# henriChevreux/distillation_trajectories

Hardware: AMD Instinct MI355X
Metric: trajectory-timesteps/sec (B×T U-Net fwd) at 16×16 T=50 (higher is better)
Workload: dtype f32 (fp32-accurate; convolutions: exact 3-plane bf16 operand split on bf16 MFMA with fp32 accumulate, or native fp32 MFMA, chosen per layer)

## Files before the change

### distillation_trajectories_amd/csrc/dt_conv_strip.hip

```cpp
#include <mutex>
#include <type_traits>

#include "dt_conv_epilogue.h"

namespace dt {

extern __shared__ __attribute__((aligned(16))) __bf16 strip_lds[];

template <int BM, int BN, int ABL = 0, int KC = 1, int WK = 1>
__global__ __launch_bounds__(256, KC == 1 ? 3 : 2) void conv_strip_bf16x6_kernel(const ConvParams p) {
  constexpr int WN = WK > 1 ? BN / 64 : (BM == 256 ? 1 : 2), WM = 4 / (WN * WK), NT = 256;
  constexpr int MI = BM / (32 * WM), NI = BN / (32 * WN);
  constexpr int KW = KC / WK;
  static_assert(KC % WK == 0 && MI * 32 * WM == BM && NI * 32 * WN == BN && (WK == 1 || (MI == 2 && NI == 2)), "wave layout");
  constexpr int PLANE_B = BN * 16, STAGE_B = 3 * PLANE_B;
  constexpr int AP = BM == 256 ? 3 : (KC == 4 ? 1 : 2);
  const int halo = strip_halo(p.W, BM);
  const int R = BM + 2 * halo;
  const int RZ = (R + 7) & ~7;
  const int PLANE_A = (RZ + 8) * 16;
  __bf16 *As = strip_lds;
  __bf16 *Bs = strip_lds + KC * 3 * PLANE_A;

  const int tid = threadIdx.x, lane = tid & 63;
  const int wave = __builtin_amdgcn_readfirstlane(tid >> 6);
  const int wk = wave % WK, wm = (wave / WK) / WN, wn = (wave / WK) % WN;
  const int half = lane >> 5, l31 = lane & 31;
  const int m0 = blockIdx.x * BM, n0 = blockIdx.y * BN;
  const int HW = p.H * p.W;
  const int CC = p.cin_p >> 4;

  bool s_in[AP], s_ok[AP], s_core[AP];
  int s_off[AP], s_off2[AP], s_offb[AP], s_lds[AP];
#pragma unroll
  for (int i = 0; i < AP; ++i) {
    const int item = tid + i * NT;
    const int srow = item >> 1, hh = item & 1;
    const int m = m0 - halo + srow;
    s_in[i] = item < 2 * R;
    s_ok[i] = s_in[i] && m >= 0 && m < p.M;
    s_core[i] = s_ok[i] && srow >= halo && srow < halo + BM;
    const int mm = s_ok[i] ? m : 0;
    s_off[i] = mm * p.cin_p + hh * 8;
    s_off2[i] = mm * p.cin2_p + hh * 8;
    s_offb[i] = mm * p.b_stride + hh * 8;
    s_lds[i] = srow * 16 + ((hh ^ ((srow >> 3) & 1)) << 3);
  }
  constexpr bool B_ALL = WK > 1 && BN * 4 == NT;
  constexpr int NB = B_ALL ? KC * 3 / 2 : KC * 3, SB = B_ALL ? 2 : 1;
  static_assert(!B_ALL || (KC * 3) % 2 == 0, "weight staging");
  const bool b_thread = B_ALL || tid < BN * 2;
  const int bt = B_ALL ? (tid & (BN * 2 - 1)) : tid, bsub = B_ALL ? tid / (BN * 2) : 0;
  const size_t w_plane = (size_t)p.n_p * 16;
  const __bf16 *wbase = reinterpret_cast<const __bf16 *>(p.w) + (size_t)n0 * 16 + bt * 8 + bsub * w_plane;
  const __bf16 *wbase2 = reinterpret_cast<const __bf16 *>(p.w2) + (size_t)n0 * 16 + bt * 8 + bsub * w_plane;
  const int b_lds = bsub * PLANE_B + bt * 8;

  int a_row[MI];
  unsigned a_mask[MI];
#pragma unroll
  for (int mi = 0; mi < MI; ++mi) {
    const int row_i = wm * (MI * 32) + mi * 32 + l31;
    const int m = m0 + row_i;
    a_row[mi] = row_i + halo;
    unsigned mask = 0;
    if (m < p.M) {
      const int rem = m % HW;
      const int y = rem / p.W, x = rem - y * p.W;
#pragma unroll
      for (int t = 0; t < 9; ++t) {
        const int yy = y + t / 3 - 1, xx = x + t % 3 - 1;
        if (yy >= 0 && yy < p.H && xx >= 0 && xx < p.W) mask |= 1u << t;
      }
    }
    a_mask[mi] = mask;
  }
  int b_frag[NI];
#pragma unroll
  for (int ni = 0; ni < NI; ++ni) {
    const int row = wn * (NI * 32) + ni * 32 + l31;
    b_frag[ni] = row * 16 + ((half ^ ((row >> 3) & 1)) << 3);
  }

  f32x16 acc[MI][NI];
#pragma unroll
  for (int mi = 0; mi < MI; ++mi)
#pragma unroll
    for (int ni = 0; ni < NI; ++ni)
#pragma unroll
      for (int r = 0; r < 16; ++r) acc[mi][ni][r] = 0.f;

  const int n_main = (CC + p.splits * KC - 1) / (p.splits * KC);
  const int cc0 = blockIdx.z * n_main * KC;
  const int CC2 = p.cin2_p >> 4;
  const int n_chunks = n_main + (p.in2 ? (CC2 + KC - 1) / KC : 0);

  f32x4 sa0[KC][AP], sa1[KC][AP];
  u32x4 rb[NB];
  auto load_strip = [&](int ch) __attribute__((always_inline)) {
#pragma unroll
    for (int kk = 0; kk < KC; ++kk)
#pragma unroll
    for (int i = 0; i < AP; ++i) {
      sa0[kk][i] = f32x4{0.f, 0.f, 0.f, 0.f}; sa1[kk][i] = sa0[kk][i];
      if (ch < n_main) {
        const int cc = cc0 + ch * KC + kk;
        if (s_ok[i] && cc < CC) {
          const float *src = (p.in_b && cc >= p.cc_a) ? p.in_b + s_offb[i] + (cc - p.cc_a) * 16 : p.in + s_off[i] + cc * 16;
          sa0[kk][i] = *reinterpret_cast<const f32x4 *>(src);
          sa1[kk][i] = *reinterpret_cast<const f32x4 *>(src + 4);
        }
      } else if (s_core[i] && (ch - n_main) * KC + kk < CC2) {
        const int c2 = (ch - n_main) * KC + kk;
        const float *src = (p.in2_b && c2 >= p.cc_a) ? p.in2_b + s_offb[i] + (c2 - p.cc_a) * 16 : p.in2 + s_off2[i] + c2 * 16;
        sa0[kk][i] = *reinterpret_cast<const f32x4 *>(src);
        sa1[kk][i] = *reinterpret_cast<const f32x4 *>(src + 4);
      }
    }
  };
  auto write_strip = [&]() __attribute__((always_inline)) {
#pragma unroll
    for (int kk = 0; kk < KC; ++kk)
#pragma unroll
    for (int i = 0; i < AP; ++i)
      if (s_in[i]) {
        bf16x8 p1, p2, p3;
        split8(sa0[kk][i], sa1[kk][i], p1, p2, p3);
        __bf16 *A = As + kk * 3 * PLANE_A;
        *reinterpret_cast<bf16x8 *>(A + s_lds[i]) = p1;
        *reinterpret_cast<bf16x8 *>(A + PLANE_A + s_lds[i]) = p2;
        *reinterpret_cast<bf16x8 *>(A + 2 * PLANE_A + s_lds[i]) = p3;
      }
  };
  const size_t tap_stride = (size_t)p.ccw * 3 * w_plane, group_stride = (size_t)KC * 3 * w_plane;
  const __bf16 *wrun = wbase + (size_t)cc0 * 3 * w_plane;
  enum { ADV_NONE = 0, ADV_TAP, ADV_GROUP, ADV_SKIP0, ADV_SKIP };
  auto load_b = [&](int adv) __attribute__((always_inline)) {
    if (adv == ADV_TAP) wrun += tap_stride;
    else if (adv == ADV_GROUP) wrun = wrun - 8 * tap_stride + group_stride;
    else if (adv == ADV_SKIP0) wrun = wbase2;
    else if (adv == ADV_SKIP) wrun += group_stride;
    if (b_thread) {
      const __bf16 *wt = ABL == 6 ? wbase : wrun;
#pragma unroll
      for (int i = 0; i < NB; ++i)
        rb[i] = *reinterpret_cast<const u32x4 *>(wt + (SB * i) * w_plane);
    }
  };
  auto write_b = [&](int stage) __attribute__((always_inline)) {
    if (b_thread) {
      __bf16 *B = Bs + stage * KC * STAGE_B;
#pragma unroll
      for (int i = 0; i < NB; ++i) *reinterpret_cast<u32x4 *>(B + (SB * i) * PLANE_B + b_lds) = rb[i];
    }
  };

  constexpr bool DB = WK > 1 && ABL == 0;
  bf16x8 fbn[KW][NI][3];
  auto load_bd = [&](int adv) __attribute__((always_inline)) {
    if (adv == ADV_TAP) wrun += tap_stride;
    else if (adv == ADV_GROUP) wrun = wrun - 8 * tap_stride + group_stride;
    else if (adv == ADV_SKIP0) wrun = wbase2;
    else if (adv == ADV_SKIP) wrun += group_stride;
    const __bf16 *wt = wrun - (bt * 8 + bsub * w_plane);
#pragma unroll
    for (int kw = 0; kw < KW; ++kw)
#pragma unroll
      for (int ni = 0; ni < NI; ++ni)
#pragma unroll
        for (int pl = 0; pl < 3; ++pl)
          fbn[kw][ni][pl] = *reinterpret_cast<const bf16x8 *>(wt + ((wk * KW + kw) * 3 + pl) * w_plane + b_frag[ni]);
  };

  const long long tl0 = p.ablate == 8 ? wall_clock64() : 0;
  load_strip(0);
  if (DB) load_bd(ADV_NONE); else load_b(ADV_NONE);
  if (tid < 48 * KC) *reinterpret_cast<u32x4 *>(As + (tid >> 4) * PLANE_A + RZ * 16 + (tid & 15) * 8) = u32x4{0u, 0u, 0u, 0u};
  write_strip();
  if (!DB) write_b(0);
  __syncthreads();

  unsigned long long ph[4] = {0, 0, 0, 0}, ts = 0;
  auto stamp = [&](int seg) __attribute__((always_inline)) {
    if (ABL != 9) return;
    unsigned long long t;
    __builtin_amdgcn_sched_barrier(0);
    asm volatile("s_memtime %0\n\ts_waitcnt lgkmcnt(0)" : "=s"(t) :: "memory");
    __builtin_amdgcn_sched_barrier(0);
    if (seg >= 0) ph[seg] += t - ts;
    ts = t;
  };
  stamp(-1);
  const long long tl_pro = p.ablate == 8 ? wall_clock64() : 0;
  int step = 0;
  bool stage_next_strip = true;
  auto do_step = [&](auto TT, int ch, bool first_tap, bool last_tap, bool next_chunk, int adv) __attribute__((always_inline)) {
    constexpr int tt = decltype(TT)::value;
    const bool more = !last_tap || next_chunk;
    if (first_tap && next_chunk && stage_next_strip && ABL != 5) load_strip(ch + 1);
    bf16x8 fbc[KW][NI][3];
    if (DB) {
#pragma unroll
      for (int kw = 0; kw < KW; ++kw)
#pragma unroll
        for (int ni = 0; ni < NI; ++ni)
#pragma unroll
          for (int pl = 0; pl < 3; ++pl) fbc[kw][ni][pl] = fbn[kw][ni][pl];
      if (more) load_bd(adv);
    } else if (more && ABL != 2) load_b(adv);
    {
      int wv = p.W;
      asm volatile("" : "+s"(wv));
      const int shift = (tt / 3 - 1) * wv + (tt % 3 - 1);
      int a_e[MI];
#pragma unroll
      for (int mi = 0; mi < MI; ++mi) {
        int row0 = a_row[mi];
        asm volatile("" : "+v"(row0));
        const int srow = row0 + shift;
        const int lrow = ((a_mask[mi] >> tt) & 1u) ? srow : RZ + (srow & 7);
        a_e[mi] = lrow * 16 + ((half ^ ((srow >> 3) & 1)) << 3);
      }
#pragma unroll
      for (int kw = 0; kw < KW; ++kw) {
        const int kk = wk * KW + kw;
        const __bf16 *A = As + kk * 3 * PLANE_A;
        const __bf16 *B = Bs + ((step & 1) * KC + kk) * STAGE_B;
        bf16x8 fb[NI][3];
        const u32x4 fake = {(unsigned)lane * 0x01010101u + (unsigned)a_e[0], 0x3f803f80u, (unsigned)step, 0x3c003c00u};
#pragma unroll
        for (int ni = 0; ni < NI; ++ni)
#pragma unroll
          for (int pl = 0; pl < 3; ++pl)
            fb[ni][pl] = DB ? fbc[kw][ni][pl]
                            : ((ABL == 4) ? __builtin_bit_cast(bf16x8, fake) : *reinterpret_cast<const bf16x8 *>(B + pl * PLANE_B + b_frag[ni]));
#pragma unroll
        for (int mi = 0; mi < MI; ++mi) {
          bf16x8 fa[3];
#pragma unroll
          for (int pl = 0; pl < 3; ++pl)
            fa[pl] = (ABL == 4) ? __builtin_bit_cast(bf16x8, fake) : *reinterpret_cast<const bf16x8 *>(A + pl * PLANE_A + a_e[mi]);
#pragma unroll
          for (int ni = 0; ni < NI; ++ni) {
            f32x16 c = acc[mi][ni];
            if (ABL == 3) {
              asm volatile("" :: "v"(fa[0]), "v"(fa[1]), "v"(fa[2]), "v"(fb[ni][0]), "v"(fb[ni][1]), "v"(fb[ni][2]));
              continue;
            }
            c = __builtin_amdgcn_mfma_f32_32x32x16_bf16(fa[2], fb[ni][0], c, 0, 0, 0);
            c = __builtin_amdgcn_mfma_f32_32x32x16_bf16(fa[1], fb[ni][1], c, 0, 0, 0);
            c = __builtin_amdgcn_mfma_f32_32x32x16_bf16(fa[0], fb[ni][2], c, 0, 0, 0);
            c = __builtin_amdgcn_mfma_f32_32x32x16_bf16(fa[1], fb[ni][0], c, 0, 0, 0);
            c = __builtin_amdgcn_mfma_f32_32x32x16_bf16(fa[0], fb[ni][1], c, 0, 0, 0);
            c = __builtin_amdgcn_mfma_f32_32x32x16_bf16(fa[0], fb[ni][0], c, 0, 0, 0);
            acc[mi][ni] = c;
          }
        }
      }
    }
    stamp(0);
    if (ABL == 9) { asm volatile("s_waitcnt vmcnt(0)" ::: "memory"); stamp(1); }
    if (!DB && more && ABL != 2) write_b((step + 1) & 1);
    stamp(2);
    const bool restage = last_tap && next_chunk && stage_next_strip && ABL != 5;
    if (restage) {
      __syncthreads();
      write_strip();
    }
    if (DB ? restage : (ABL != 1 || last_tap)) __syncthreads();
    stamp(3);
    ++step;
  };

  constexpr bool DIRECT = MI * KW <= 2 && KC >= 2 && ABL == 0;
  f32x4 ga0[KW][MI][2], ga1[KW][MI][2];
  const int n_skip = p.in2 ? (CC2 + KC - 1) / KC : 0;
  auto load_a = [&](f32x4 (&g)[KW][MI][2], int s2) __attribute__((always_inline)) {
#pragma unroll
    for (int kw = 0; kw < KW; ++kw)
#pragma unroll
      for (int mi = 0; mi < MI; ++mi) {
        const int c2 = s2 * KC + wk * KW + kw;
        const int m = m0 + wm * (MI * 32) + mi * 32 + l31;
        g[kw][mi][0] = f32x4{0.f, 0.f, 0.f, 0.f}; g[kw][mi][1] = g[kw][mi][0];
        if (m < p.M && c2 < CC2) {
          const float *src = (p.in2_b && c2 >= p.cc_a) ? p.in2_b + (size_t)m * p.b_stride + (c2 - p.cc_a) * 16 + half * 8
                                                       : p.in2 + (size_t)m * p.cin2_p + c2 * 16 + half * 8;
          g[kw][mi][0] = *reinterpret_cast<const f32x4 *>(src);
          g[kw][mi][1] = *reinterpret_cast<const f32x4 *>(src + 4);
        }
      }
  };
  auto skip_step = [&](f32x4 (&g)[KW][MI][2], int s2) __attribute__((always_inline)) {
    const bool more = s2 + 1 < n_skip;
    bf16x8 fbc[KW][NI][3];
    if (DB) {
#pragma unroll
      for (int kw = 0; kw < KW; ++kw)
#pragma unroll
        for (int ni = 0; ni < NI; ++ni)
#pragma unroll
          for (int pl = 0; pl < 3; ++pl) fbc[kw][ni][pl] = fbn[kw][ni][pl];
      if (more) load_bd(ADV_SKIP);
    } else if (more) load_b(ADV_SKIP);
#pragma unroll
    for (int kw = 0; kw < KW; ++kw) {
      const int kk = wk * KW + kw;
      const __bf16 *B = Bs + ((step & 1) * KC + kk) * STAGE_B;
      bf16x8 fb[NI][3];
#pragma unroll
      for (int ni = 0; ni < NI; ++ni)
#pragma unroll
        for (int pl = 0; pl < 3; ++pl) fb[ni][pl] = DB ? fbc[kw][ni][pl] : *reinterpret_cast<const bf16x8 *>(B + pl * PLANE_B + b_frag[ni]);
#pragma unroll
      for (int mi = 0; mi < MI; ++mi) {
        bf16x8 fa[3];
        split8(g[kw][mi][0], g[kw][mi][1], fa[0], fa[1], fa[2]);
#pragma unroll
        for (int ni = 0; ni < NI; ++ni) {
          f32x16 c = acc[mi][ni];
          c = __builtin_amdgcn_mfma_f32_32x32x16_bf16(fa[2], fb[ni][0], c, 0, 0, 0);
          c = __builtin_amdgcn_mfma_f32_32x32x16_bf16(fa[1], fb[ni][1], c, 0, 0, 0);
          c = __builtin_amdgcn_mfma_f32_32x32x16_bf16(fa[0], fb[ni][2], c, 0, 0, 0);
          c = __builtin_amdgcn_mfma_f32_32x32x16_bf16(fa[1], fb[ni][0], c, 0, 0, 0);
          c = __builtin_amdgcn_mfma_f32_32x32x16_bf16(fa[0], fb[ni][1], c, 0, 0, 0);
          c = __builtin_amdgcn_mfma_f32_32x32x16_bf16(fa[0], fb[ni][0], c, 0, 0, 0);
          acc[mi][ni] = c;
        }
      }
    }
    if (s2 + 2 < n_skip) load_a(g, s2 + 2);
    if (!DB) {
      if (more) write_b((step + 1) & 1);
      __syncthreads();
    }
    ++step;
  };

  const int prio_grp = ((blockIdx.x + gridDim.x * (blockIdx.y + gridDim.y * blockIdx.z)) >> 8) & 1;
  const bool use_prio = p.ablate != 7 && gridDim.x * gridDim.y * gridDim.z <= 512;
  for (int ch = 0; ch < n_main; ++ch) {
    if (use_prio) {
      if ((ch ^ prio_grp) & 1) __builtin_amdgcn_s_setprio(1);
      else __builtin_amdgcn_s_setprio(0);
    }
    const bool next_chunk = ch + 1 < ((WK > 1 && p.in2) ? n_main : n_chunks);
    if (DIRECT && WK == 1 && p.in2 && ch + 1 == n_main) {
      stage_next_strip = false;
      load_a(ga0, 0);
      if (n_skip > 1) load_a(ga1, 1);
    }
    do_step(std::integral_constant<int, 0>{}, ch, true, false, next_chunk, ADV_TAP);
    do_step(std::integral_constant<int, 1>{}, ch, false, false, next_chunk, ADV_TAP);
    do_step(std::integral_constant<int, 2>{}, ch, false, false, next_chunk, ADV_TAP);
    do_step(std::integral_constant<int, 3>{}, ch, false, false, next_chunk, ADV_TAP);
    do_step(std::integral_constant<int, 4>{}, ch, false, false, next_chunk, ADV_TAP);
    do_step(std::integral_constant<int, 5>{}, ch, false, false, next_chunk, ADV_TAP);
    do_step(std::integral_constant<int, 6>{}, ch, false, false, next_chunk, ADV_TAP);
    do_step(std::integral_constant<int, 7>{}, ch, false, false, next_chunk, ADV_TAP);
    do_step(std::integral_constant<int, 8>{}, ch, false, true, next_chunk, ch + 1 < n_main ? ADV_GROUP : ADV_SKIP0);
    if (ch + 1 == n_main && p.in2) {
      if constexpr (WK == 1) {
        conv_midpoint<MI, NI>(p, acc, n0, wn, l31);
      } else {
        constexpr int P = BN + 4, COPY = WM * 32 * P;
        float *red = reinterpret_cast<float *>(strip_lds);
#pragma unroll
        for (int mi = 0; mi < MI; ++mi) {
          if (mi || DB) __syncthreads();
#pragma unroll
          for (int ni = 0; ni < NI; ++ni)
#pragma unroll
            for (int r = 0; r < 16; ++r)
              red[wk * COPY + (wm * 32 + 4 * half + (r & 3) + 8 * (r >> 2)) * P + wn * (NI * 32) + ni * 32 + l31] = acc[mi][ni][r];
          __syncthreads();
#pragma unroll
          for (int ni = 0; ni < NI; ++ni)
#pragma unroll
            for (int r = 0; r < 16; ++r) {
              const float *src = red + (wm * 32 + 4 * half + (r & 3) + 8 * (r >> 2)) * P + wn * (NI * 32) + ni * 32 + l31;
              float v = src[0];
#pragma unroll
              for (int c = 1; c < WK; ++c) v += src[c * COPY];
              acc[mi][ni][r] = wk == 0 ? v : 0.f;
            }
        }
        if (wk == 0) conv_midpoint<MI, NI>(p, acc, n0, wn, l31);
        __syncthreads();
        if (DB) load_bd(ADV_SKIP0); else load_b(ADV_SKIP0);
        if (DIRECT) {
          load_a(ga0, 0);
          if (n_skip > 1) load_a(ga1, 1);
        } else {
          load_strip(n_main);
          if (tid < 48 * KC) *reinterpret_cast<u32x4 *>(As + (tid >> 4) * PLANE_A + RZ * 16 + (tid & 15) * 8) = u32x4{0u, 0u, 0u, 0u};
          write_strip();
        }
        if (!DB) write_b(step & 1);
        __syncthreads();
      }
    }
  }
  __builtin_amdgcn_s_setprio(0);
  if (DIRECT) {
    for (int s2 = 0; s2 < n_skip; s2 += 2) {
      skip_step(ga0, s2);
      if (s2 + 1 < n_skip) skip_step(ga1, s2 + 1);
    }
  } else {
    for (int ch = n_main; ch < n_chunks; ++ch)
      do_step(std::integral_constant<int, 4>{}, ch, true, true, ch + 1 < n_chunks, ADV_SKIP);
  }
  const long long tl1 = p.ablate == 8 ? wall_clock64() : 0;
  conv_epilogue<MI, NI, WM, WK>(p, acc, reinterpret_cast<float *>(strip_lds), m0, n0, wm, wn, half, l31, wk);
  if (ABL == 9) {
    if (lane == 0) {
      unsigned long long *rec = reinterpret_cast<unsigned long long *>(p.slab) + 8 * (4 * (blockIdx.x + gridDim.x * (blockIdx.y + gridDim.y * blockIdx.z)) + wave);
      rec[0] = ph[0]; rec[1] = ph[1]; rec[2] = ph[2]; rec[3] = ph[3]; rec[4] = (unsigned long long)step;
    }
  }
  if (p.ablate == 8 && p.splits == 1) {
    __syncthreads();
    if (tid == 0) {
      long long *rec = reinterpret_cast<long long *>(p.slab) + 4 * (blockIdx.x + gridDim.x * blockIdx.y);
      rec[0] = tl0; rec[1] = tl_pro; rec[2] = tl1; rec[3] = wall_clock64();
    }
  }
}

int launch_conv_strip(const ConvParams &p_in, hipStream_t s) {
  ConvParams p = p_in;
  const int bm = p.bm, bn = p.bn, kind = p.kind;
  const int kc = strip_kc(kind, bm, bn);
  dim3 grid((p.M + bm - 1) / bm, p.n_p / bn, p.splits);
  size_t lds = strip_lds_bytes(p.W, bm, bn, kind);
  p.dup_stage2 = 0;
  if (p.n_dup == 2 && p.pool_out) {
    const size_t rows1 = bm == 256 || kc == 4 || (kind == KIND_STRIPK && bm == 128) ? 128 : 64;
    const size_t rows2 = bm == 256 ? 128 : (bm == 128 ? 64 : 32);
    const size_t need = (rows1 + (kind == KIND_STRIPK ? rows2 : rows1)) * (bn + 4) * sizeof(float);
    if (need <= strip_lds_limit(kind)) {
      p.dup_stage2 = 1;
      if (need > lds) lds = need;
    }
  }
#ifdef DT_TOOLS
  if (p.ablate && p.ablate != 7 && p.ablate != 8 && bm == 128 && bn == 128) {
    switch (p.ablate) {
      case 1: conv_strip_bf16x6_kernel<128, 128, 1><<<grid, 256, lds, s>>>(p); break;
      case 2: conv_strip_bf16x6_kernel<128, 128, 2><<<grid, 256, lds, s>>>(p); break;
      case 3: conv_strip_bf16x6_kernel<128, 128, 3><<<grid, 256, lds, s>>>(p); break;
      case 4: conv_strip_bf16x6_kernel<128, 128, 4><<<grid, 256, lds, s>>>(p); break;
      case 5: conv_strip_bf16x6_kernel<128, 128, 5><<<grid, 256, lds, s>>>(p); break;
      case 6: conv_strip_bf16x6_kernel<128, 128, 6><<<grid, 256, lds, s>>>(p); break;
      case 9: conv_strip_bf16x6_kernel<128, 128, 9><<<grid, 256, lds, s>>>(p); break;
      default: return DT_E_ARG;
    }
    DT_LAUNCH_CHECK();
    return DT_OK;
  }
#endif
  if (kind != KIND_STRIP) {
    static std::once_flag attr_once;
    static int attr_status = DT_OK;
    std::call_once(attr_once, [] {
      const void *fns[8] = {reinterpret_cast<const void *>(&conv_strip_bf16x6_kernel<64, 128, 0, 2, 2>),
                            reinterpret_cast<const void *>(&conv_strip_bf16x6_kernel<64, 64, 0, 4, 4>),
                            reinterpret_cast<const void *>(&conv_strip_bf16x6_kernel<128, 64, 0, 2, 2>),
                            reinterpret_cast<const void *>(&conv_strip_bf16x6_kernel<256, 64, 0, 2>),
                            reinterpret_cast<const void *>(&conv_strip_bf16x6_kernel<128, 128, 0, 2>),
                            reinterpret_cast<const void *>(&conv_strip_bf16x6_kernel<128, 64, 0, 2>),
                            reinterpret_cast<const void *>(&conv_strip_bf16x6_kernel<64, 128, 0, 2>),
                            reinterpret_cast<const void *>(&conv_strip_bf16x6_kernel<64, 64, 0, 2>)};
      for (const void *f : fns) {
        const hipError_t e = hipFuncSetAttribute(f, hipFuncAttributeMaxDynamicSharedMemorySize, 98304);
        if (e != hipSuccess) attr_status = (int)e;
      }
    });
    if (attr_status != DT_OK) return attr_status;
    if (kind == KIND_STRIPK && bn == 128) conv_strip_bf16x6_kernel<64, 128, 0, 2, 2><<<grid, 256, lds, s>>>(p);
    else if (kind == KIND_STRIPK && bm == 64) conv_strip_bf16x6_kernel<64, 64, 0, 4, 4><<<grid, 256, lds, s>>>(p);
    else if (kind == KIND_STRIPK) conv_strip_bf16x6_kernel<128, 64, 0, 2, 2><<<grid, 256, lds, s>>>(p);
    else if (bm == 256) conv_strip_bf16x6_kernel<256, 64, 0, 2><<<grid, 256, lds, s>>>(p);
    else if (bm == 128 && bn == 128) conv_strip_bf16x6_kernel<128, 128, 0, 2><<<grid, 256, lds, s>>>(p);
    else if (bm == 128) conv_strip_bf16x6_kernel<128, 64, 0, 2><<<grid, 256, lds, s>>>(p);
    else if (bn == 128) conv_strip_bf16x6_kernel<64, 128, 0, 2><<<grid, 256, lds, s>>>(p);
    else conv_strip_bf16x6_kernel<64, 64, 0, 2><<<grid, 256, lds, s>>>(p);
    DT_LAUNCH_CHECK();
    return DT_OK;
  }
  if (bm == 256) conv_strip_bf16x6_kernel<256, 64><<<grid, 256, lds, s>>>(p);
  else if (bm == 128 && bn == 128) conv_strip_bf16x6_kernel<128, 128><<<grid, 256, lds, s>>>(p);
  else if (bm == 128) conv_strip_bf16x6_kernel<128, 64><<<grid, 256, lds, s>>>(p);
  else if (bn == 128) conv_strip_bf16x6_kernel<64, 128><<<grid, 256, lds, s>>>(p);
  else conv_strip_bf16x6_kernel<64, 64><<<grid, 256, lds, s>>>(p);
  DT_LAUNCH_CHECK();
  return DT_OK;
}

}
```

Measured before the change: 346,300.

## Double-buffer the activation strip in the 64x64 K-split strip conv kernel

Adds an SDB variant of the K-split strip convolution that keeps two LDS copies of the bf16-split activation strip. The next chunk's strip is loaded and written in two halves at taps 0/3 and 3/6, so the restage barrier no longer has to write the whole strip serially. It also computes weight and activation addresses with 32-bit byte offsets from a running base to cut address arithmetic. The cost is twice the strip LDS footprint, which may lower occupancy, and an environment variable can turn the variant off.

Result: no change. 347,700 (median of 6 runs) (+0.4%).

```diff
diff --git a/distillation_trajectories_amd/csrc/dt_conv_strip.hip b/distillation_trajectories_amd/csrc/dt_conv_strip.hip
--- a/distillation_trajectories_amd/csrc/dt_conv_strip.hip
+++ b/distillation_trajectories_amd/csrc/dt_conv_strip.hip
@@ -1,3 +1,4 @@
+#include <cstdlib>
 #include <mutex>
 #include <type_traits>
 
@@ -7,7 +8,7 @@
 
 extern __shared__ __attribute__((aligned(16))) __bf16 strip_lds[];
 
-template <int BM, int BN, int ABL = 0, int KC = 1, int WK = 1>
+template <int BM, int BN, int ABL = 0, int KC = 1, int WK = 1, bool SDB = false>
 __global__ __launch_bounds__(256, KC == 1 ? 3 : 2) void conv_strip_bf16x6_kernel(const ConvParams p) {
   constexpr int WN = WK > 1 ? BN / 64 : (BM == 256 ? 1 : 2), WM = 4 / (WN * WK), NT = 256;
   constexpr int MI = BM / (32 * WM), NI = BN / (32 * WN);
@@ -19,6 +20,8 @@
   const int R = BM + 2 * halo;
   const int RZ = (R + 7) & ~7;
   const int PLANE_A = (RZ + 8) * 16;
+  static_assert(!SDB || (WK > 1 && ABL == 0 && KC % 2 == 0), "double-buffered strip: K split only");
+  constexpr int KH = SDB ? KC / 2 : KC;
   __bf16 *As = strip_lds;
   __bf16 *Bs = strip_lds + KC * 3 * PLANE_A;
 
@@ -95,38 +98,44 @@
   const int CC2 = p.cin2_p >> 4;
   const int n_chunks = n_main + (p.in2 ? (CC2 + KC - 1) / KC : 0);
 
-  f32x4 sa0[KC][AP], sa1[KC][AP];
+  f32x4 sa0[KH][AP], sa1[KH][AP];
   u32x4 rb[NB];
-  auto load_strip = [&](int ch) __attribute__((always_inline)) {
-#pragma unroll
-    for (int kk = 0; kk < KC; ++kk)
+  auto load_strip = [&](int ch, int h = 0) __attribute__((always_inline)) {
+#pragma unroll
+    for (int k = 0; k < KH; ++k)
 #pragma unroll
     for (int i = 0; i < AP; ++i) {
-      sa0[kk][i] = f32x4{0.f, 0.f, 0.f, 0.f}; sa1[kk][i] = sa0[kk][i];
+      const int kk = h * KH + k;
+      sa0[k][i] = f32x4{0.f, 0.f, 0.f, 0.f}; sa1[k][i] = sa0[k][i];
       if (ch < n_main) {
         const int cc = cc0 + ch * KC + kk;
         if (s_ok[i] && cc < CC) {
-          const float *src = (p.in_b && cc >= p.cc_a) ? p.in_b + s_offb[i] + (cc - p.cc_a) * 16 : p.in + s_off[i] + cc * 16;
-          sa0[kk][i] = *reinterpret_cast<const f32x4 *>(src);
-          sa1[kk][i] = *reinterpret_cast<const f32x4 *>(src + 4);
+          const bool from_b = p.in_b && cc >= p.cc_a;
+          const float *src = from_b ? p.in_b + s_offb[i] + (cc - p.cc_a) * 16 : p.in + s_off[i] + cc * 16;
+          if constexpr (SDB) {
+            const float *base = from_b ? p.in_b + (cc - p.cc_a) * 16 : p.in + cc * 16;
+            src = reinterpret_cast<const float *>(reinterpret_cast<const char *>(base) + (unsigned)(from_b ? s_offb[i] : s_off[i]) * 4u);
+          }
+          sa0[k][i] = *reinterpret_cast<const f32x4 *>(src);
+          sa1[k][i] = *reinterpret_cast<const f32x4 *>(src + 4);
         }
       } else if (s_core[i] && (ch - n_main) * KC + kk < CC2) {
         const int c2 = (ch - n_main) * KC + kk;
         const float *src = (p.in2_b && c2 >= p.cc_a) ? p.in2_b + s_offb[i] + (c2 - p.cc_a) * 16 : p.in2 + s_off2[i] + c2 * 16;
-        sa0[kk][i] = *reinterpret_cast<const f32x4 *>(src);
-        sa1[kk][i] = *reinterpret_cast<const f32x4 *>(src + 4);
-      }
-    }
-  };
-  auto write_strip = [&]() __attribute__((always_inline)) {
-#pragma unroll
-    for (int kk = 0; kk < KC; ++kk)
+        sa0[k][i] = *reinterpret_cast<const f32x4 *>(src);
+        sa1[k][i] = *reinterpret_cast<const f32x4 *>(src + 4);
+      }
+    }
+  };
+  auto write_strip = [&](int buf = 0, int h = 0) __attribute__((always_inline)) {
+#pragma unroll
+    for (int k = 0; k < KH; ++k)
 #pragma unroll
     for (int i = 0; i < AP; ++i)
       if (s_in[i]) {
         bf16x8 p1, p2, p3;
-        split8(sa0[kk][i], sa1[kk][i], p1, p2, p3);
-        __bf16 *A = As + kk * 3 * PLANE_A;
+        split8(sa0[k][i], sa1[k][i], p1, p2, p3);
+        __bf16 *A = As + (buf * KC + h * KH + k) * 3 * PLANE_A;
         *reinterpret_cast<bf16x8 *>(A + s_lds[i]) = p1;
         *reinterpret_cast<bf16x8 *>(A + PLANE_A + s_lds[i]) = p2;
         *reinterpret_cast<bf16x8 *>(A + 2 * PLANE_A + s_lds[i]) = p3;
@@ -157,7 +166,26 @@
 
   constexpr bool DB = WK > 1 && ABL == 0;
   bf16x8 fbn[KW][NI][3];
+  const __bf16 *wtu = reinterpret_cast<const __bf16 *>(p.w) + (size_t)n0 * 16 + (size_t)cc0 * 3 * w_plane;
+  unsigned b_off[NI];
+#pragma unroll
+  for (int ni = 0; ni < NI; ++ni) b_off[ni] = (unsigned)b_frag[ni] * sizeof(__bf16);
   auto load_bd = [&](int adv) __attribute__((always_inline)) {
+    if constexpr (SDB) {
+      if (adv == ADV_TAP) wtu += tap_stride;
+      else if (adv == ADV_GROUP) wtu = wtu - 8 * tap_stride + group_stride;
+      else if (adv == ADV_SKIP0) wtu = reinterpret_cast<const __bf16 *>(p.w2) + (size_t)n0 * 16;
+      else if (adv == ADV_SKIP) wtu += group_stride;
+#pragma unroll
+      for (int kw = 0; kw < KW; ++kw)
+#pragma unroll
+        for (int pl = 0; pl < 3; ++pl) {
+          const char *wt = reinterpret_cast<const char *>(wtu + ((wk * KW + kw) * 3 + pl) * w_plane);
+#pragma unroll
+          for (int ni = 0; ni < NI; ++ni) fbn[kw][ni][pl] = *reinterpret_cast<const bf16x8 *>(wt + b_off[ni]);
+        }
+      return;
+    }
     if (adv == ADV_TAP) wrun += tap_stride;
     else if (adv == ADV_GROUP) wrun = wrun - 8 * tap_stride + group_stride;
     else if (adv == ADV_SKIP0) wrun = wbase2;
@@ -175,8 +203,13 @@
   const long long tl0 = p.ablate == 8 ? wall_clock64() : 0;
   load_strip(0);
   if (DB) load_bd(ADV_NONE); else load_b(ADV_NONE);
-  if (tid < 48 * KC) *reinterpret_cast<u32x4 *>(As + (tid >> 4) * PLANE_A + RZ * 16 + (tid & 15) * 8) = u32x4{0u, 0u, 0u, 0u};
+  for (int z = tid; z < 48 * KC * (SDB ? 2 : 1); z += NT)
+    *reinterpret_cast<u32x4 *>(As + (z >> 4) * PLANE_A + RZ * 16 + (z & 15) * 8) = u32x4{0u, 0u, 0u, 0u};
   write_strip();
+  if constexpr (SDB) {
+    load_strip(0, 1);
+    write_strip(0, 1);
+  }
   if (!DB) write_b(0);
   __syncthreads();
 
@@ -197,7 +230,13 @@
   auto do_step = [&](auto TT, int ch, bool first_tap, bool last_tap, bool next_chunk, int adv) __attribute__((always_inline)) {
     constexpr int tt = decltype(TT)::value;
     const bool more = !last_tap || next_chunk;
-    if (first_tap && next_chunk && stage_next_strip && ABL != 5) load_strip(ch + 1);
+    if constexpr (SDB) {
+      if (next_chunk && tt == 3) write_strip((ch + 1) & 1, 0);
+      if (next_chunk && tt == 6) write_strip((ch + 1) & 1, 1);
+      if (next_chunk && (tt == 0 || tt == 3)) load_strip(ch + 1, tt == 3);
+    } else if (first_tap && next_chunk && stage_next_strip && ABL != 5) {
+      load_strip(ch + 1);
+    }
     bf16x8 fbc[KW][NI][3];
     if (DB) {
 #pragma unroll
@@ -224,7 +263,7 @@
 #pragma unroll
       for (int kw = 0; kw < KW; ++kw) {
         const int kk = wk * KW + kw;
-        const __bf16 *A = As + kk * 3 * PLANE_A;
+        const __bf16 *A = As + ((SDB ? (ch & 1) * KC : 0) + kk) * 3 * PLANE_A;
         const __bf16 *B = Bs + ((step & 1) * KC + kk) * STAGE_B;
         bf16x8 fb[NI][3];
         const u32x4 fake = {(unsigned)lane * 0x01010101u + (unsigned)a_e[0], 0x3f803f80u, (unsigned)step, 0x3c003c00u};
@@ -263,6 +302,11 @@
     if (!DB && more && ABL != 2) write_b((step + 1) & 1);
     stamp(2);
     const bool restage = last_tap && next_chunk && stage_next_strip && ABL != 5;
+    if (SDB && restage) {
+      __syncthreads();
+      ++step;
+      return;
+    }
     if (restage) {
       __syncthreads();
       write_strip();
@@ -428,6 +472,16 @@
   }
 }
 
+static size_t stripk_sdb_lds(const ConvParams &p, size_t lds) {
+  const char *env = getenv("DT_STRIPK_STRIP_DB");
+  if (env && env[0] == '0' && env[1] == 0) return 0;
+  const size_t R = p.bm + 2 * strip_halo(p.W, p.bm);
+  const size_t two = (size_t)2 * strip_kc(KIND_STRIPK, p.bm, p.bn) * 3 * (((R + 7) & ~(size_t)7) + 8) * 16 * sizeof(__bf16);
+  const size_t need = two > lds ? two : lds;
+  const size_t row = (size_t)(p.cin_p > p.b_stride ? p.cin_p : p.b_stride) * sizeof(float);
+  return need <= strip_lds_limit(KIND_STRIPK) && (size_t)p.M * row <= 0xffffffffu ? need : 0;
+}
+
 int launch_conv_strip(const ConvParams &p_in, hipStream_t s) {
   ConvParams p = p_in;
   const int bm = p.bm, bn = p.bn, kind = p.kind;
@@ -464,7 +518,8 @@
     static std::once_flag attr_once;
     static int attr_status = DT_OK;
     std::call_once(attr_once, [] {
-      const void *fns[8] = {reinterpret_cast<const void *>(&conv_strip_bf16x6_kernel<64, 128, 0, 2, 2>),
+      const void *fns[9] = {reinterpret_cast<const void *>(&conv_strip_bf16x6_kernel<64, 128, 0, 2, 2>),
+                            reinterpret_cast<const void *>(&conv_strip_bf16x6_kernel<64, 64, 0, 4, 4, true>),
                             reinterpret_cast<const void *>(&conv_strip_bf16x6_kernel<64, 64, 0, 4, 4>),
                             reinterpret_cast<const void *>(&conv_strip_bf16x6_kernel<128, 64, 0, 2, 2>),
                             reinterpret_cast<const void *>(&conv_strip_bf16x6_kernel<256, 64, 0, 2>),
@@ -478,6 +533,13 @@
       }
     });
     if (attr_status != DT_OK) return attr_status;
+    if (kind == KIND_STRIPK && bm == 64 && bn == 64) {
+      if (const size_t lds2 = stripk_sdb_lds(p, lds)) {
+        conv_strip_bf16x6_kernel<64, 64, 0, 4, 4, true><<<grid, 256, lds2, s>>>(p);
+        DT_LAUNCH_CHECK();
+        return DT_OK;
+      }
+    }
     if (kind == KIND_STRIPK && bn == 128) conv_strip_bf16x6_kernel<64, 128, 0, 2, 2><<<grid, 256, lds, s>>>(p);
     else if (kind == KIND_STRIPK && bm == 64) conv_strip_bf16x6_kernel<64, 64, 0, 4, 4><<<grid, 256, lds, s>>>(p);
     else if (kind == KIND_STRIPK) conv_strip_bf16x6_kernel<128, 64, 0, 2, 2><<<grid, 256, lds, s>>>(p);
```
